# wenet-e2e/wetts

Measured on AMD Instinct MI355X. Metric: audio samples/sec + RTF @22.05 kHz, VITS-Baker, 1/2/4/8 MI355X, higher is better.
Workload: dtype f32

## Files before the change

### wetts_amd/build.py

```python
import hashlib
import os
import subprocess
import sys

HERE = os.path.dirname(os.path.abspath(__file__))
CSRC = os.path.join(HERE, "csrc")
LIBDIR = os.path.join(HERE, "lib")
LIB = os.path.join(LIBDIR, "libwetts_hip.so")
SOURCES = ["conv_mfma.hip", "gemm_pw.hip", "conv_small.hip", "conv_bf16.hip", "resblock16.hip", "resblock2_stage16.hip", "wn16.hip", "qconv_u8.hip", "resblock32.hip", "resblock_chain32.hip", "kernels.hip", "dds_fused.hip", "attention.hip", "mas.hip", "align.hip", "losses.hip", "duration_loss.hip", "stft.hip", "discriminator.hip", "mrd.hip", "model.hip"]
BENCH_SOURCES = ["bench_conv.hip"]
BENCH_LIB = os.path.join(LIBDIR, "libwetts_bench.so")
HEADERS = ["bench_abi.h", "qconv_u8.h", "common.h", "kernels.h", "conv_bf16.h", "conv16_dev.h", "resblock32.h", os.path.join("..", "..", "include", "wetts_hip.h"),
           os.path.join("..", "..", "include", "wetts_vits_model.hpp"),
           os.path.join("..", "..", "tests", "native", "vits_model_main.cpp")]
FLAGS = ["--offload-arch=gfx950", "-O3", "-std=c++17", "-fPIC", "-Wall", "-Wno-unused-function"]


def _hipcc():
    for c in (os.environ.get("HIPCC"), "/opt/rocm/bin/hipcc", "hipcc"):
        if c and (os.path.isabs(c) and os.path.exists(c) or not os.path.isabs(c)):
            return c
    raise RuntimeError("hipcc not found")


def _digest():
    h = hashlib.sha256()
    for f in SOURCES + BENCH_SOURCES + HEADERS:
        with open(os.path.join(CSRC, f), "rb") as fh:
            h.update(fh.read())
    h.update(" ".join(FLAGS).encode())
    return h.hexdigest()


def _obj_digest(src):
    h = hashlib.sha256()
    for f in [src] + [x for x in HEADERS if x.endswith(".h")]:
        with open(os.path.join(CSRC, f), "rb") as fh:
            h.update(fh.read())
    h.update(" ".join(FLAGS).encode())
    return h.hexdigest()


def build(force=False, verbose=True):
    os.makedirs(LIBDIR, exist_ok=True)
    stamp = os.path.join(LIBDIR, "build.sha256")
    dig = _digest()
    if not force and os.path.exists(LIB) and os.path.exists(stamp):
        if open(stamp).read().strip() == dig:
            return LIB
    hipcc = _hipcc()
    objs = []
    procs = []
    for src in SOURCES + BENCH_SOURCES:
        obj = os.path.join(LIBDIR, src.replace(".hip", ".o"))
        objs.append(obj)
        odig = _obj_digest(src)
        ostamp = obj + ".sha256"
        if not force and os.path.exists(obj) and os.path.exists(ostamp) and open(ostamp).read().strip() == odig:
            continue
        if os.path.exists(ostamp):
            os.remove(ostamp)
        cmd = [hipcc] + FLAGS + ["-c", os.path.join(CSRC, src), "-o", obj]
        if verbose:
            print("[wetts_amd.build]", " ".join(cmd), flush=True)
        procs.append((src, ostamp, odig, subprocess.Popen(cmd, stdout=subprocess.PIPE, stderr=subprocess.STDOUT)))
# ... 38 lines not shown
```

### wetts_amd/csrc/common.h

```cpp
#pragma once
#include <hip/hip_runtime.h>
#include <stdint.h>
#include <stdio.h>
#include <string>

#include <string.h>

#include "../../include/wetts_hip.h"

namespace wetts {

void set_error(const char* fmt, ...);

#define WETTS_HIP_CHECK(expr)                                                        \
  do {                                                                               \
    hipError_t _e = (expr);                                                          \
    if (_e != hipSuccess) {                                                          \
      ::wetts::set_error("%s failed: %s (%s:%d)", #expr, hipGetErrorString(_e),      \
                         __FILE__, __LINE__);                                        \
      return WETTS_E_HIP;                                                            \
    }                                                                                \
  } while (0)

static inline bool lds_opt_in(const void* kernel, signed char* state) {
// ... 31 lines not shown
    if (_r != WETTS_OK) return _r; \
  } while (0)

constexpr int kConvCK = 16;

enum InAct { IN_NONE = 0, IN_LRELU = 1 };
enum OutAct { OUT_NONE = 0, OUT_RELU = 1, OUT_GELU = 2, OUT_GATE = 3 };
__device__ __forceinline__ float wn_gate(float ta, float sa) { return tanhf(ta) * (1.f / (1.f + expf(-sa))); }

__device__ __forceinline__ float div_small_const(float v, float d, float c) {
  const float q = v * c;
  const float r = __builtin_fmaf(-d, q, v);
  return __builtin_fmaf(r, c, q);
}

__device__ __forceinline__ bool mrf_div_fast(float d) { return d == 3.f || d == 2.f; }
__device__ __forceinline__ float mrf_div(float v, float d, float dinv, bool fast) {
  return fast ? div_small_const(v, d, dinv) : v / d;
}

struct ConvParams {
  const float* x;
  int64_t x_bs, x_cs;
  int Cin, Tin;
  int vec_in;
  int in_rev_base;
  int in_act;
  float in_slope;
  const float* in_mask;
  int64_t in_mask_stride;
  const float* wpk;
  const float* bias;
  const float* bias_b;
  int64_t bias_b_stride;
  int M, N;
  int ktaps, dil, pad;
  int off_lo, span;
  int nchunks;
  float* out;
  int64_t o_bs, o_cs;
  int Tout;
  int up_shift;
  int up, up_pad;
  int out_act;
  const float* out_mask;
  int64_t out_mask_stride;
  const float* res;
  int64_t r_bs, r_cs;
  int accum;
  float out_div;
  int B;
  int tag;
  int k_rows_padded;
  const int64_t* lens;
  int len_mul;
  float* wn_h;
  float* wn_skip;
  const float* wn_mask;
  int64_t wn_mask_stride;
  int wn_H, wn_last, wn_first;
};

inline ConvParams conv_io(const float* x, int Cin, int T, float* out, int Cout, int B) {
  ConvParams p;
  memset(&p, 0, sizeof(p));
  p.x = x;
  p.x_bs = (int64_t)Cin * T;
  p.x_cs = T;
  p.Tin = T;
  p.in_rev_base = -1;
  p.in_act = IN_NONE;
  p.in_slope = 0.f;
  p.out = out;
  p.o_bs = (int64_t)Cout * T;
  p.o_cs = T;
  p.Tout = T;
  p.out_act = OUT_NONE;
  p.out_div = 1.f;
  p.B = B;
  return p;
}

struct PackedConv {
  float* wpk = nullptr;
  const float* bias = nullptr;
  int M = 0, Cin = 0, ktaps = 0, dil = 1, pad = 0;
  int up = 0, up_pad = 0;
  int Cout = 0;
  int k_orig = 0;
  int off_lo = 0, span = 0, nchunks = 0;
  int gate_H = 0;
};

int32_t pack_conv_weight(const float* w_dev, const float* bias_dev, int Cout, int Cin, int k,
                         int dil, int pad, int transposed, int up, hipStream_t stream,
                         PackedConv* out, int rev_in = 0, int gate_H = 0);
void free_packed(PackedConv* pc);

int32_t launch_conv(const PackedConv& pc, ConvParams p, hipStream_t stream);
bool pw_gemm_eligible(const PackedConv& pc, const ConvParams& p);
int32_t launch_pw_gemm(const PackedConv& pc, const ConvParams& p, hipStream_t stream, int variant);
int32_t launch_conv_group(const PackedConv* const* pcs, const ConvParams* ps, int n, hipStream_t stream,
                          int* launches = nullptr);

int conv_variant();
void set_conv_variant(int v);
int32_t launch_conv_small(const ConvParams& p, hipStream_t stream, bool* taken);
struct SmallConvScope {
  explicit SmallConvScope(int max_tiles);
  ~SmallConvScope();
  int prev;
};

inline int cdiv(int a, int b) { return (a + b - 1) / b; }
inline int64_t align_up(int64_t v, int64_t a) { return (v + a - 1) / a * a; }

inline int device_cus() {
  static int cus = 0;
  if (cus == 0) {
    int dev = 0, n = 0;
    cus = (hipGetDevice(&dev) == hipSuccess &&
           hipDeviceGetAttribute(&n, hipDeviceAttributeMultiprocessorCount, dev) == hipSuccess && n > 0) ? n : 256;
  }
  return cus;
}

}
```

### wetts_amd/csrc/conv_mfma.hip

```cpp
#include <stdlib.h>

#include "common.h"

namespace wetts {

typedef float f32x16 __attribute__((ext_vector_type(16)));
typedef float f32x4v __attribute__((ext_vector_type(4)));
constexpr int kBufRsrcDword3 = 0x00020000;

__device__ __forceinline__ float lrelu2(float x, float slope) {
  const float m = x * slope;
  float r;
  asm("v_max_f32 %0, %1, %2" : "=v"(r) : "v"(x), "v"(m));
  return r;
}

__global__ void pack_conv_weight_kernel(const float* __restrict__ w, float* __restrict__ out,
                                        int M, int Cin, int Cout, int k, int ktaps, int up,
                                        int transposed, int rev_in, int gate_H, int G, int64_t total) {
  int64_t idx = (int64_t)blockIdx.x * blockDim.x + threadIdx.x;
  if (idx >= total) return;
  int s = (int)(idx & 3);
  int lane = (int)((idx >> 2) & 63);
  int64_t rest = idx >> 8;
  int g = (int)(rest % G);
  int mt32 = (int)(rest / G);
  int kstep = g * 4 + s;
  int per_chunk = ktaps * 8;
  int chunk = kstep / per_chunk;
  int within = kstep % per_chunk;
  int tap = within / 8;
  int pair = within % 8;
  int ci = chunk * kConvCK + pair * 2 + (lane >> 5);
  int row = mt32 * 32 + (lane & 31);
  float v = 0.f;
  if (row < M && ci < Cin) {
    if (!transposed) {
      const int src = gate_H > 0 ? (row & 1) * gate_H + (row >> 1) : row;
      v = w[((int64_t)src * Cin + (rev_in ? Cin - 1 - ci : ci)) * k + tap];
    } else {
      int co = row / up, ph = row % up;
      int kk = ph + tap * up;
      if (kk < k) v = w[((int64_t)ci * Cout + co) * k + kk];
    }
  }
  out[idx] = v;
}

int32_t pack_conv_weight(const float* w_dev, const float* bias_dev, int Cout, int Cin, int k,
                         int dil, int pad, int transposed, int up, hipStream_t stream,
                         PackedConv* pc, int rev_in, int gate_H) {
  WETTS_REQUIRE(gate_H == 0 || (!transposed && Cout == 2 * gate_H), "gate packing needs a Conv1d with 2 * gate_H rows");
  pc->gate_H = gate_H;
  pc->Cin = Cin;
  pc->Cout = Cout;
// ... 645 lines not shown
    total += (int64_t)cdiv(gp.p[j].N, NT) * cdiv(gp.p[j].M, MT) * gp.p[j].B;
  }
  gp.first[gp.n] = (int)total;
  WETTS_REQUIRE(total > 0 && total < (1ll << 31), "conv group grid size");
  const size_t lds = (size_t)2 * kConvCK * (conv_has_fixed_stride(NT) ? conv_fixed_stride(NT) : ((NT + max_span + 3 + 3) & ~3)) *
                     sizeof(float);
  hipLaunchKernelGGL((conv_mfma_group_kernel<MB, NB, WM, WN, 1>), dim3((unsigned)total), dim3(256), lds, stream, gp);
  WETTS_LAUNCH_CHECK();
  return WETTS_OK;
}

int32_t launch_conv_group(const PackedConv* const* pcs, const ConvParams* ps, int n, hipStream_t stream,
                          int* launches) {
  if (launches) *launches = n;
  if (n <= 0) return WETTS_OK;
  ConvGroupParams gp;
  memset(&gp, 0, sizeof(gp));
  bool ok = n >= 2 && n <= kConvGroupMax && conv_variant() == 0;
  int order[kConvGroupMax] = {0, 1, 2};
  if (ok) {
    for (int a = 0; a < n; ++a)
      for (int b = a + 1; b < n; ++b)
        if (pcs[order[b]]->ktaps > pcs[order[a]]->ktaps) { int t = order[a]; order[a] = order[b]; order[b] = t; }
  }
  int max_span = 0;
  for (int j = 0; j < n && ok; ++j) {
    gp.p[j] = ps[order[j]];
    WETTS_TRY(prepare_conv(*pcs[order[j]], gp.p[j]));
    const ConvParams& q = gp.p[j];
    ok = q.up == 0 && q.out_act == OUT_NONE && q.out_mask == nullptr && q.out_div == 1.f && q.tag && conv_fast_ok(q) &&
         q.M == gp.p[0].M && q.N == gp.p[0].N && q.B == gp.p[0].B && q.Cin == gp.p[0].Cin && q.lens == gp.p[0].lens;
    if (q.span > max_span) max_span = q.span;
  }
  gp.n = n;
  if (ok) {
    const ConvParams& q = gp.p[0];
    const int64_t cols = (int64_t)q.N * q.B;
    auto nblk = [&](int mt, int nt) { return (int64_t)cdiv(q.M, mt) * cdiv(q.N, nt) * q.B; };
    if (q.M >= 128 && cols >= 4096 && nblk(128, 128) >= 384) {
      if (launches) *launches = 1;
      return launch_group_cfg<1, 4, 4, 1>(gp, max_span, stream);
    }
    if (q.M > 32 && q.M < 128 && cols >= 8192 && nblk(64, 256) >= 384) {
      if (launches) *launches = 1;
      return launch_group_cfg<1, 4, 2, 2>(gp, max_span, stream);
    }
  }
  for (int j = 0; j < n; ++j) WETTS_TRY(launch_conv(*pcs[j], ps[j], stream));
  return WETTS_OK;
}

int32_t launch_conv(const PackedConv& pc, ConvParams p, hipStream_t stream) {
  WETTS_TRY(prepare_conv(pc, p));
  if (conv_variant() == 0 && p.lens == nullptr) {
    bool taken = false;
    WETTS_TRY(launch_conv_small(p, stream, &taken));
    if (taken) return WETTS_OK;
  }
  {
    const int v = conv_variant();
    if ((v == 0 || (v >= 7 && v <= 9)) && pw_gemm_eligible(pc, p)) return launch_pw_gemm(pc, p, stream, v);
  }
  const int64_t cols = (int64_t)p.N * p.B;
  switch (conv_variant()) {
    case 2: return launch_cfg<1, 2, 4, 1>(p, stream);
    case 3: return launch_cfg<1, 4, 2, 2>(p, stream);
    case 4: return launch_cfg<1, 2, 2, 2>(p, stream);
    case 5: return launch_cfg<1, 1, 2, 2>(p, stream);
    case 6: return launch_cfg<1, 4, 4, 1>(p, stream);
    default: break;
  }
  auto nblk = [&](int mt, int nt) { return (int64_t)cdiv(p.M, mt) * cdiv(p.N, nt) * p.B; };
  constexpr int64_t kFill = 384;
  if (p.M >= 128 && cols >= 4096) {
    const int64_t n128 = nblk(128, 128);
    const int kCUs = device_cus();
    if (n128 >= 4 * kCUs) return launch_cfg<1, 4, 4, 1>(p, stream);
    auto cost = [&](int64_t blocks, int area, double eff) {
      return (blocks < kCUs ? 4.0 : 1.0) * (double)((blocks + kCUs - 1) / kCUs) * area / eff;
    };
    const double c128 = cost(n128, 128 * 128, 1.18), c64w = cost(nblk(64, 128), 64 * 128, 1.07),
                 c64 = cost(nblk(64, 64), 64 * 64, 1.0);
    if (c128 <= c64w && c128 <= c64) return launch_cfg<1, 4, 4, 1>(p, stream);
    if (c64w <= c64) return launch_cfg<1, 2, 2, 2>(p, stream);
    return launch_cfg<1, 1, 2, 2>(p, stream);
  }
  if (p.M > 32 && cols >= 8192) {
    if (nblk(64, 256) >= kFill) return launch_cfg<1, 4, 2, 2>(p, stream);
    return launch_cfg<1, 1, 2, 2>(p, stream);
  }
  if (p.M <= 32 && cols >= 8192 && p.ktaps >= 5) return launch_cfg<1, 4, 1, 4>(p, stream);
  if (p.M <= 32 && cols >= 8192) return launch_cfg<1, 2, 1, 4>(p, stream);
  return launch_cfg<1, 1, 2, 2>(p, stream);
}

}
```

### wetts_amd/csrc/gemm_pw.hip

```cpp
#include "common.h"

namespace wetts {

typedef float f32x16 __attribute__((ext_vector_type(16)));
typedef float f32x4v __attribute__((ext_vector_type(4)));
constexpr int kPwRsrcDword3 = 0x00020000;

struct PwParams {
  const float* x;
  int64_t x_bs;
  int x_cs, K, N;
  const float* wpk;
  int64_t wpk_bytes;
  int G;
  const float* bias;
  const float* bias_b;
  int64_t bias_b_stride;
  int M;
  float* out;
  int64_t o_bs;
  int o_cs;
  const float* res;
  int64_t r_bs;
  int r_cs;
// ... 187 lines not shown

template <int CKS, int NBMAX, bool TAG = false>
__global__ __launch_bounds__(256) __attribute__((amdgpu_waves_per_eu(4, 4))) void pw_gemm_kernel(const PwParams p) {
  extern __shared__ __attribute__((aligned(16))) float smem[];
  const int tid = threadIdx.x;
  const int lane = tid & 63;
  const int wave = __builtin_amdgcn_readfirstlane(tid >> 6);
  int bid = blockIdx.x;
  const int total = gridDim.x;
  if ((total & 7) == 0) bid = (bid & 7) * (total >> 3) + (bid >> 3);
  const int part = bid % p.S;
  bid /= p.S;
  const int mtile = bid % p.mtiles;
  const int b = __builtin_amdgcn_readfirstlane(bid / p.mtiles);
  __amdgpu_buffer_rsrc_t rsx = __builtin_amdgcn_make_buffer_rsrc(
      const_cast<float*>(p.x + (int64_t)b * p.x_bs), 0, __builtin_amdgcn_readfirstlane(p.K * p.x_cs * 4), kPwRsrcDword3);
  __amdgpu_buffer_rsrc_t rsw = __builtin_amdgcn_make_buffer_rsrc(const_cast<float*>(p.wpk), 0, (int)p.wpk_bytes,
                                                                 kPwRsrcDword3);
  int u = part * p.upb;
  const int u1 = min(u + p.upb, p.U);
  while (u < u1) {
    const int w = u1 - u;
    if (NBMAX >= 4 && w >= 4) {
      pw_pass<CKS, NBMAX, (NBMAX >= 4 ? 4 : NBMAX)>(p, smem, b, mtile, u * 32, lane, wave, rsx, rsw);
      u += 4;
    } else if (NBMAX >= 2 && w >= 2) {
      pw_pass<CKS, NBMAX, (NBMAX >= 2 ? 2 : NBMAX)>(p, smem, b, mtile, u * 32, lane, wave, rsx, rsw);
      u += 2;
    } else {
      pw_pass<CKS, NBMAX, 1>(p, smem, b, mtile, u * 32, lane, wave, rsx, rsw);
      u += 1;
    }
  }
}

bool pw_gemm_eligible(const PackedConv& pc, const ConvParams& p) {
  if (pc.ktaps != 1 || pc.up != 0 || pc.pad != 0) return false;
  if (p.in_act != IN_NONE || p.in_mask != nullptr || p.in_rev_base >= 0 || p.lens != nullptr) return false;
  if (p.accum || p.out_div != 1.f || p.out_act == OUT_GATE) return false;
  if (p.wn_skip && ((p.wn_H % 32) != 0 || (pc.M % 32) != 0 || p.res || p.out_act != OUT_NONE || p.out_mask ||
                    p.wn_mask_stride < p.Tout))
    return false;
  if (p.res && (p.out_act != OUT_NONE || p.out_mask)) return false;
  if (p.res && (pc.M % 32) != 0) return false;
  if ((int64_t)pc.M * p.o_cs * 4 >= (1ll << 31) || (p.res && (int64_t)pc.M * p.r_cs * 4 >= (1ll << 31))) return false;
  if (((pc.Cin % 16) != 0 && !p.k_rows_padded) || pc.Cin < 32) return false;
  if ((p.x_cs & 3) != 0 || (p.x_bs & 3) != 0 || (reinterpret_cast<uintptr_t>(p.x) & 15) != 0) return false;
  if (p.Tin > p.x_cs || p.x_cs < 4 || p.Tout != p.Tin) return false;
  if ((int64_t)pc.nchunks * 16 * p.x_cs * 4 >= (1ll << 31)) return false;
  if (p.k_rows_padded && p.x_bs < (int64_t)pc.nchunks * 16 * p.x_cs) return false;
  return true;
}

static void pw_schedule(int strips, int U, int K, int slots, int* S_out, int* upb_out) {
  const int cus = device_cus();
  double best = 1e30;
  int bestS = 1;
  for (int S = 1; S <= U; ++S) {
    const int upb = cdiv(U, S);
    if (S > 1 && cdiv(U, S - 1) == upb) continue;
    const int64_t blocks = (int64_t)strips * cdiv(U, upb);
    const int64_t per_cu = cdiv(blocks, cus);
    const int npass = upb / 4 + ((upb % 4) >= 2 ? 1 : 0) + ((upb % 4) & 1);
    double block_cost = (double)upb * K + npass * (0.12 * K + 96.0);
    block_cost += ((upb % 4) >= 2 ? 2.0 * K * 0.08 : 0.0) + ((upb % 4) & 1 ? 1.0 * K * 0.20 : 0.0);
    const int resident = (int)(per_cu < slots ? per_cu : slots);
    const double eff = resident >= 3 ? 1.0 : resident == 2 ? 0.85 : 0.6;
    const double cost = (double)per_cu * block_cost / eff;
    if (cost < best * 0.999) {
      best = cost;
      bestS = cdiv(U, upb);
    }
  }
  *S_out = bestS;
  *upb_out = cdiv(U, bestS);
}

template <int CKS, int NBMAX>
static int32_t launch_pw(const PwParams& p, int64_t blocks, hipStream_t stream, bool tag = false) {
  const size_t lds = PwLds<CKS, NBMAX>::kBytes;
  static signed char opt_in[64] = {};
  if (lds > 64 * 1024 && !lds_opt_in(reinterpret_cast<const void*>(&pw_gemm_kernel<CKS, NBMAX>), opt_in)) {
    set_error("pw_gemm_kernel: the device refused the %zu-byte dynamic LDS opt-in", lds);
    return WETTS_E_HIP;
  }
  if (tag && lds <= 64 * 1024)
    hipLaunchKernelGGL((pw_gemm_kernel<CKS, NBMAX, true>), dim3((unsigned)blocks), dim3(256), lds, stream, p);
  else
    hipLaunchKernelGGL((pw_gemm_kernel<CKS, NBMAX>), dim3((unsigned)blocks), dim3(256), lds, stream, p);
  WETTS_LAUNCH_CHECK();
  return WETTS_OK;
}

int32_t launch_pw_gemm(const PackedConv& pc, const ConvParams& cp, hipStream_t stream, int variant) {
  PwParams p;
  memset(&p, 0, sizeof(p));
  p.x = cp.x;
  p.x_bs = cp.x_bs;
  p.x_cs = (int)cp.x_cs;
  p.K = pc.nchunks * 16;
  p.N = cp.Tout;
  p.wpk = pc.wpk;
  p.G = pc.nchunks * 2;
  p.mtiles = cdiv(pc.M, 128);
  p.wpk_bytes = (int64_t)p.mtiles * 4 * p.G * 1024;
  p.bias = pc.bias;
  p.bias_b = cp.bias_b;
// ... 34 lines not shown
```

### wetts_amd/csrc/model.hip

```cpp
#include <stdarg.h>
#include <stdlib.h>
#include <string.h>

#include <map>
#include <string>
#include <vector>

#include "common.h"
#include "conv_bf16.h"
#include "resblock32.h"
#include "qconv_u8.h"
#include "kernels.h"

namespace wetts {

static thread_local char g_err[512] = "";

void set_error(const char* fmt, ...) {
  va_list ap;
  va_start(ap, fmt);
  vsnprintf(g_err, sizeof(g_err), fmt, ap);
  va_end(ap);
}

struct TensorSpec {
  std::string name;
  int64_t shape[4];
  int64_t offset, numel;
  int dil = 1, pad = 0, transposed = 0, up = 0;
  int bias = -1;
};

struct Layout {
  std::vector<TensorSpec> specs;
  std::map<std::string, int> index;
  int64_t total = 0;
  void add(const std::string& name, int64_t d0, int64_t d1 = 0, int64_t d2 = 0, int64_t d3 = 0) {
    TensorSpec t;
    t.name = name;
    t.shape[0] = d0; t.shape[1] = d1; t.shape[2] = d2; t.shape[3] = d3;
    t.numel = d0 * (d1 ? d1 : 1) * (d2 ? d2 : 1) * (d3 ? d3 : 1);
    t.offset = total;
    total += (t.numel + 63) / 64 * 64;
    index[name] = (int)specs.size();
    specs.push_back(t);
  }
  void add_conv(const std::string& prefix, int Cout, int Cin, int k, int dil = 1, int pad = 0, int transposed = 0,
                int up = 0, bool bias = true) {
    const int w = (int)specs.size();
    add(prefix + ".weight", transposed ? Cin : Cout, transposed ? Cout : Cin, k);
    specs[w].dil = dil; specs[w].pad = pad; specs[w].transposed = transposed; specs[w].up = up;
    if (bias) {
      specs[w].bias = w + 1;
      add(prefix + ".bias", Cout);
    }
  }
  const TensorSpec* find(const std::string& name) const {
    auto it = index.find(name);
    return it == index.end() ? nullptr : &specs[it->second];
  }
};

static const float* tensor(const Layout& L, const float* blob, const std::string& name) {
// ... 306 lines not shown
  PackedConv conv_pre;
  std::vector<PackedConv> ups;
  std::vector<RB> rbs;
  const float* conv_post_w = nullptr;
  const float *dec_cond_w = nullptr, *dec_cond_b = nullptr;
  int hop = 1;
  PackedConv v_in, v_out, v_istft, v_istft_onnx;
  mutable int istft_mode = 0;
  std::vector<ConvNeXt> v_layers;
  const float *v_npre_g = nullptr, *v_npre_b = nullptr, *v_npost_g = nullptr, *v_npost_b = nullptr;
  std::vector<float*> v_owned;
  mutable bool mrf_timing = false;
  mutable std::vector<std::pair<hipEvent_t, hipEvent_t>> mrf_events;
  mutable int64_t mrf_launches = 0;
  mutable int32_t mrf_calls = 0;
  mutable double mrf_bytes = 0;
  mutable int dec_precision = 0;
  mutable int dec_unfused = 0;
  mutable int dec_serial = 0;
  int fuse32_lds = 160 * 1024;
  int fuse32_kmax128 = 11;
  int fuse32_maxc = 32;
  int fuse32_kmax = 99;
  int fuse32_kwide = 3;
  int fuse2_maxc = 128;
  int fuse_min_blocks = 128;
  int small_max_tiles = 256;
  int chain_whole_waste_pct = 15;
  int chain_whole_maxc = 64;
  int chain_pair_maxc = 32;
  int chain_pair_kmax = 3;
  int fuse2_waste_pct = 20;
  mutable int flow_precision = 0;
  mutable std::vector<std::vector<PackedConvB>> b_wn_in, b_wn_rs;
  mutable PackedConvB b_post;
  mutable float* b_post_wpad = nullptr;
  mutable PackedQConv q_pre, q_cond, q_post;
  mutable std::vector<std::vector<PackedQConv>> q_c1, q_c2;
  mutable bool q_packed = false;
  mutable int flow_packed_prec = 0, dec_packed_prec = 0;
  mutable std::vector<PackedConvB> b_ups;
  mutable PackedConvB b_pre;
  mutable std::vector<std::vector<PackedConvB>> b_c1, b_c2;
  mutable int32_t* status_word = nullptr;
  mutable uint64_t rng_seed = 0, rng_offset = 0;
  int mrf_streams = 1;
  int mrf_fork_maxc = 1 << 20;
  int stage2_pct = 30;
  int dds_fused = 1;
  int attn_small_max_t = 128;
  int wn_gate = 1;
  int wn_fuse = 1;
  int small_fork = 1;
  int conv_groups = 1;
  hipStream_t aux_stream[WETTS_MAX_RB_KERNELS] = {};
  hipEvent_t ev_fork = nullptr, ev_chain[WETTS_MAX_RB_KERNELS] = {};
  bool fork_ok = false;

  int spec_channels = 0;
  bool post_loaded = false;
  Layout post_layout;
  float* post_blob = nullptr;
  PackedConv pe_pre, pe_proj;
  std::vector<PackedConv> pe_in, pe_rs, fwd_pre;
  const float *pe_cond_w = nullptr, *pe_cond_b = nullptr;

  bool dur_loaded = false;
  Layout dur_layout;
  float* dur_blob = nullptr;
  ConvFlowW dur_cf1;
  std::vector<ConvFlowW> dur_post_cf;
  const float *dur_post_pre_w = nullptr, *dur_post_pre_b = nullptr;
  PackedConv dur_post_proj;
  DDS dur_post_dds;
  const float *dur_qm = nullptr, *dur_qlogs = nullptr;

  const float* T(const std::string& name) const { return tensor(layout, blob, name); }
};

namespace wetts {

struct Bump {
  char* base;
  int64_t cap, off = 0;
  bool ok = true;
  Bump(void* p, int64_t c) : base((char*)p), cap(c) {}
  template <typename T>
  T* take(int64_t n) {
    int64_t bytes = align_up(n * (int64_t)sizeof(T), 256);
    if (off + bytes > cap) {
      ok = false;
      return nullptr;
    }
    T* r = (T*)(base + off);
    off += bytes;
    return r;
  }
};

struct ConvRef {
  const float *w, *b;
  int Cout, Cin, k, dil, pad, transposed, up;
};

static int32_t find_conv(const Layout& L, const float* blob, const std::string& prefix, ConvRef* r) {
  const std::string wname = prefix + ".weight";
// ... 229 lines not shown
    PackedConv* pc = g.kind == GenConv::PRE  ? &m->conv_pre
                     : g.kind == GenConv::UP ? &m->ups[g.i]
                     : g.kind == GenConv::C1 ? &m->rbs[g.n].c1[g.d]
                     : g.kind == GenConv::C2 ? &m->rbs[g.n].c2[g.d]
                                             : nullptr;
    if (pc) WETTS_TRY(load_conv(m, g.prefix, s, pc));
    if (g.kind == GenConv::UP) m->hop *= g.up;
  }
  m->conv_post_w = m->T("dec.conv_post.weight");
  m->dec_cond_w = m->T("dec.cond.weight");
  m->dec_cond_b = m->T("dec.cond.bias");
  return WETTS_OK;
}

static int64_t A256(int64_t n_floats) { return align_up(n_floats * 4, 256); }

static int64_t ws_encoder(const wetts_config_t* c, int B, int Tx) {
  const int64_t H = c->hidden_channels, F = c->filter_channels, nh = c->n_heads;
  int64_t n = 0;
  n += 5 * A256(B * H * Tx);
  n += A256(B * F * Tx);
  n += A256(B * nh * (int64_t)Tx * Tx + B * H * Tx + B * nh * (2 * c->window_size + 1) * Tx);
  n += A256(B * H * Tx);
  n += A256(B * H);
  return n;
}

static int64_t ws_sdp(const wetts_config_t* c, int B, int Tx) {
  const int64_t H = c->hidden_channels;
  return 5 * A256(B * H * Tx) + A256(B * 32 * Tx) + A256(B * 2 * Tx) + A256(B * H) + 256;
}

static int64_t ws_dp(const wetts_config_t* c, int B, int Tx) {
  const int64_t H = c->hidden_channels, Fd = c->dp_filter_channels;
  return A256(B * H * Tx) + 2 * A256(B * Fd * Tx) + A256(B * H);
}

static int64_t ws_flow(const wetts_config_t* c, int B, int Ty_) {
  const int64_t H = c->hidden_channels, I = c->inter_channels;
  const int64_t Ty = ((int64_t)Ty_ + 3) & ~3ll;
  int64_t n = 3 * A256(B * I * Ty) + A256(B * Ty) + 3 * A256(B * H * Ty) + 2 * A256(B * 2 * H * Ty) +
              A256(B * (I / 2) * Ty) + A256(B * 2 * H * c->flow_wn_layers);
  n += 2 * align_up(B * H * Ty * 2, 256) + 2 * align_up(B * 2 * H * Ty * 2, 256) + A256(B * H * Ty);
  if (c->transformer_flows != 0) {
    const int64_t He = half_enc_flows(c) ? I / 2 : H;
    n += 9 * A256(B * He * Ty) +
         A256(attn_score_elems(half_enc_flows(c) ? -1 : 4, (int)(He / 2), B, 2, Ty) + B * He * Ty +
              (int64_t)B * 2 * 9 * Ty);
  }
  return n;
}

static int64_t dec_max_elems(const wetts_config_t* c, int B, int L) {
  int64_t ch = c->upsample_initial_channel, len = L, mx = (int64_t)B * ch * len;
  for (int i = 0; i < c->n_upsamples; ++i) {
    ch /= 2;
    len *= c->upsample_rates[i];
    int64_t e = (int64_t)B * ch * len;
    if (e > mx) mx = e;
  }
  return mx;
}

static int64_t vocos_fs(int L) { return ((int64_t)L + 1 + 3) & ~3ll; }
static int64_t vocos_rows(const wetts_config_t* c) { return ((int64_t)c->istft_n_fft + 2 + 15) & ~15ll; }

static int64_t ws_vocos(const wetts_config_t* c, int B, int L) {
  const int64_t F = vocos_fs(L), VC = c->vocos_channels, VH = c->vocos_h_channels, NF = c->istft_n_fft;
  return A256(B * c->inter_channels * F) + 3 * A256(B * VC * F) + A256(B * VH * F) +
         A256(B * (NF + 2) * F) + A256(B * vocos_rows(c) * F) + A256(B * NF * F) + A256(B * VC);
}

static int64_t ws_decoder(const wetts_config_t* c, int B, int L) {
  if (c->vocoder_type == 1) return ws_vocos(c, B, L);
  const int64_t f32need = (3 + 3 * (int64_t)c->n_resblock_kernels) * A256(dec_max_elems(c, B, L)) +
                          A256((int64_t)B * c->upsample_initial_channel);
  int64_t lenmax = L;
  for (int i = 0; i < c->n_upsamples; ++i) lenmax *= c->upsample_rates[i];
  const int64_t u8need = 6 * A256(dec_max_elems(c, B, L)) + A256((int64_t)B * c->upsample_initial_channel) +
                         align_up(dec_max_elems(c, B, L) + 32 * (int64_t)B * lenmax, 256) +
                         align_up(4 * (int64_t)B * lenmax, 256) + 2048 + 16384 +
                         align_up((int64_t)B * (lenmax / 128 + 1) * 64, 256);
  return f32need > u8need ? f32need : u8need;
}

static void free_posterior(wetts_model* m) {
  free_packed(&m->pe_pre);
  free_packed(&m->pe_proj);
  for (auto* v : {&m->pe_in, &m->pe_rs, &m->fwd_pre})
    for (PackedConv& pc : *v) free_packed(&pc);
  m->pe_in.clear();
  m->pe_rs.clear();
  m->fwd_pre.clear();
  if (m->post_blob) (void)hipFree(m->post_blob);
  m->post_blob = nullptr;
  m->pe_cond_w = m->pe_cond_b = nullptr;
  m->post_layout = Layout();
  m->post_loaded = false;
}

static void free_dds(DDS* d) {
  for (int i = 0; i < 3; ++i) free_packed(&d->c1x1[i]);
}

static void free_convflow(ConvFlowW* cf) {
  free_dds(&cf->dds);
  free_packed(&cf->proj);
// ... 106 lines not shown
int32_t wetts_duration_blob_tensor_info(const wetts_config_t* cfg, int32_t index, char* name_buf, size_t name_buf_len,
                                        int64_t* offset, int64_t* numel, int64_t shape[4]) {
  WETTS_TRY(validate_config(cfg));
  Layout L;
  build_duration_layout(cfg, L);
  WETTS_REQUIRE(index >= 0 && index < (int32_t)L.specs.size(), "tensor index %d out of range", index);
  const TensorSpec& t = L.specs[index];
  WETTS_REQUIRE(name_buf && name_buf_len > t.name.size(), "name buffer too small");
  strcpy(name_buf, t.name.c_str());
  if (offset) *offset = t.offset;
  if (numel) *numel = t.numel;
  if (shape)
    for (int i = 0; i < 4; ++i) shape[i] = t.shape[i];
  return WETTS_OK;
}

int64_t wetts_duration_blob_numel(const wetts_config_t* cfg) {
  if (validate_config(cfg) != WETTS_OK) return WETTS_E_INVALID;
  Layout L;
  build_duration_layout(cfg, L);
  return L.total;
}

int32_t wetts_create(const wetts_config_t* cfg, const float* blob_dev, int64_t blob_numel,
                     void* stream, wetts_model_t** out) {
  WETTS_TRY(validate_config(cfg));
  WETTS_REQUIRE(out != nullptr && blob_dev != nullptr, "null argument");
  hipStream_t s = (hipStream_t)stream;
  wetts_model* m = new wetts_model();
  m->cfg = *cfg;
  build_layout(cfg, m->layout);
  if (blob_numel != m->layout.total) {
    set_error("blob has %lld floats, layout needs %lld", (long long)blob_numel,
              (long long)m->layout.total);
    delete m;
    return WETTS_E_INVALID;
  }
  hipError_t e = hipMalloc((void**)&m->blob, (size_t)blob_numel * sizeof(float));
  if (e != hipSuccess) {
    set_error("hipMalloc(blob) failed: %s", hipGetErrorString(e));
    delete m;
    return WETTS_E_HIP;
  }
  e = hipMemcpyAsync(m->blob, blob_dev, (size_t)blob_numel * sizeof(float),
                     hipMemcpyDeviceToDevice, s);
  int32_t r = (e == hipSuccess) ? build_model(m, s) : WETTS_E_HIP;
  {
    struct Knob { const char* name; int* field; };
    const Knob knobs[] = {
        {"stage2_pct", &m->stage2_pct}, {"dds_fused", &m->dds_fused}, {"wn_fuse", &m->wn_fuse}, {"wn_gate", &m->wn_gate},
        {"fuse2_waste_pct", &m->fuse2_waste_pct}, {"fuse_min_blocks", &m->fuse_min_blocks},
        {"chain_whole_pct", &m->chain_whole_waste_pct}, {"chain_whole_maxc", &m->chain_whole_maxc},
        {"small_max_tiles", &m->small_max_tiles}, {"attn_small_max_t", &m->attn_small_max_t},
    };
    if (const char* env = getenv("WETTS_TUNE")) {
      std::string all(env);
      size_t pos = 0;
      while (pos < all.size()) {
        size_t end = all.find(',', pos);
        if (end == std::string::npos) end = all.size();
        const std::string item = all.substr(pos, end - pos);
        const size_t eq = item.find('=');
        bool known = false;
        if (eq != std::string::npos)
          for (const Knob& k : knobs)
            if (item.compare(0, eq, k.name) == 0 && strlen(k.name) == eq) {
              *k.field = atoi(item.c_str() + eq + 1);
              known = true;
            }
        if (!known && !item.empty()) {
          set_error("WETTS_TUNE: unknown setting '%s'", item.c_str());
          r = WETTS_E_INVALID;
        }
        pos = end + 1;
      }
    }
    if (r == WETTS_OK && !m->wn_gate) {
      for (int f = 0; f < cfg->flow_n_flows && r == WETTS_OK; ++f)
        for (int i = 0; i < cfg->flow_wn_layers && r == WETTS_OK; ++i) {
          free_packed(&m->flows[f].in_layers[i]);
          r = pack(m->layout, m->blob, S("flow.flows.%d.enc.in_layers.%d", flow_key_stride(cfg) * f, i), s,
                   &m->flows[f].in_layers[i]);
        }
    }
    if (m->mrf_streams < 1) m->mrf_streams = 1;
    if (m->mrf_streams > cfg->n_resblock_kernels) m->mrf_streams = cfg->n_resblock_kernels;
    m->fork_ok = hipEventCreateWithFlags(&m->ev_fork, hipEventDisableTiming) == hipSuccess && m->ev_fork;
    for (int j = 0; j < cfg->n_resblock_kernels; ++j) {
      if (hipEventCreateWithFlags(&m->ev_chain[j], hipEventDisableTiming) != hipSuccess || !m->ev_chain[j]) m->fork_ok = false;
      if (j > 0)
        if (hipStreamCreateWithFlags(&m->aux_stream[j], hipStreamNonBlocking) != hipSuccess || !m->aux_stream[j]) m->fork_ok = false;
    }
    (void)hipGetLastError();
  }
  if (r == WETTS_OK) {
    e = hipStreamSynchronize(s);
    if (e != hipSuccess) {
      set_error("weight packing failed: %s", hipGetErrorString(e));
      r = WETTS_E_HIP;
    }
  }
  if (r != WETTS_OK) {
    wetts_destroy(m);
    return r;
  }
  *out = m;
// ... 1226 lines not shown
        WETTS_TRY(launch_resblock_pair32(rb.c1[d], rb.c2[d], pp, s));
        count(1, 2 + accum);
      } else {
        ConvParams p2 = conv_io(chain_buf[j][2], ch, len, outp[j], ch, B);
        p2.in_act = IN_LRELU;
        p2.in_slope = 0.1f;
        p2.res = rx[j];
        p2.r_bs = (int64_t)ch * len;
        p2.r_cs = len;
        p2.accum = accum;
        p2.out_div = odiv;
        p2.tag = 1;
        p2.lens = lens;
        p2.len_mul = spf;
        if (last_d || m->dec_unfused) {
          WETTS_TRY(launch_conv(rb.c2[d], p2, s));
          count(1, 3 + accum);
        } else {
          g2[n2] = &rb.c2[d];
          p2s[n2++] = p2;
        }
      }
      rx[j] = outp[j];
    }
    if (n2 > 0) {
      int nl = 0;
      WETTS_TRY(launch_conv_group(g2, p2s, n2, s, &nl));
      count(nl, 3.0 * n2);
    }
  }
  return WETTS_OK;
}

static int32_t run_hifigan(const wetts_model* m, const float* z, int64_t z_bs, int64_t z_cs,
                           const float* y_mask, int64_t mask_stride, const float* g, int B, int L,
                           float* audio, void* workspace, int64_t workspace_bytes, hipStream_t s,
                           DecTiming* tm, const int64_t* lens = nullptr) {
  const wetts_config_t* c = &m->cfg;
  const int I = c->inter_channels, C0 = c->upsample_initial_channel;
  const int64_t mx = dec_max_elems(c, B, L);
  Bump ws(workspace, workspace_bytes);
  float* bx = ws.take<float>(mx);
  float* bt = ws.take<float>(mx);
  float* bs = ws.take<float>(mx);
  float* chain_buf[WETTS_MAX_RB_KERNELS][3];
  for (int j = 0; j < c->n_resblock_kernels; ++j)
    for (int q = 0; q < 3; ++q) chain_buf[j][q] = ws.take<float>(mx);
  float* cond = ws.take<float>((int64_t)B * C0);
  if (!ws.ok) {
    set_error("hifigan: workspace too small (need %lld bytes)",
              (long long)ws_decoder(c, B, L));
    return WETTS_E_WORKSPACE;
  }
  {
    ConvParams p = conv_io(z, I, L, bx, C0, B);
    p.x_bs = z_bs;
    p.x_cs = z_cs;
    if (y_mask) {
      p.in_mask = y_mask;
      p.in_mask_stride = mask_stride;
    }
    if (has_g(c) && g) {
      WETTS_TRY(k_cond_linear(g, m->dec_cond_w, m->dec_cond_b, B, C0, c->gin_channels, cond, s));
      p.bias_b = cond;
      p.bias_b_stride = C0;
    }
    p.lens = lens;
    p.len_mul = 1;
    WETTS_TRY(launch_conv(m->conv_pre, p, s));
  }
  int ch = C0, len = L;
  int spf = 1;
  float* x = bx;
  float* xs = bs;
  const int nk = c->n_resblock_kernels, nd = c->n_resblock_dilations;
  for (int i = 0; i < c->n_upsamples; ++i) {
    const int u = c->upsample_rates[i];
    {
      ConvParams p = conv_io(x, ch, len, bt, ch / 2, B);
      p.in_act = IN_LRELU;
      p.in_slope = 0.1f;
      p.Tout = len * u;
      p.o_bs = (int64_t)(ch / 2) * len * u;
      p.o_cs = (int64_t)len * u;
      p.lens = lens;
      p.len_mul = spf;
      WETTS_TRY(launch_conv(m->ups[i], p, s));
    }
    ch /= 2;
    len *= u;
    spf *= u;
    float* xu = bt;
    float* xsum = (x == bx) ? bs : bx;
    (void)xs;
    if (tm && tm->on) WETTS_HIP_CHECK(hipEventRecord(tm->e0, s));
    hipEvent_t lv0 = nullptr, lv1 = nullptr;
    if (m->mrf_timing) {
      WETTS_HIP_CHECK(hipEventCreate(&lv0));
      WETTS_HIP_CHECK(hipEventCreate(&lv1));
      WETTS_HIP_CHECK(hipEventRecord(lv0, s));
    }
    const bool small_stage = !lens && (int64_t)cdiv(ch, 64) * cdiv(len, 64) * B <= m->small_max_tiles;
    const int nstreams = !m->fork_ok ? 1 : (c->resblock == 1 && ((m->small_fork && small_stage) || (ch <= m->mrf_fork_maxc && !m->dec_serial))) ? nk : m->mrf_streams;
    const bool forked = nstreams > 1;
    if (forked) WETTS_HIP_CHECK(hipEventRecord(m->ev_fork, s));
    const bool chain_addr_ok = (int64_t)ch * len * 4 < (int64_t)INT32_MAX;
    const bool grouped = c->resblock == 1 && !forked && m->conv_groups;
    if (grouped) WETTS_TRY(run_stage_rb1_grouped(m, i, xu, xsum, chain_buf, ch, len, spf, B, lens, tm, s));
    for (int j = 0; j < (grouped ? 0 : nk); ++j) {
      const RB& rb = m->rbs[i * nk + j];
      hipStream_t sj = (forked && j > 0 && j < nstreams) ? m->aux_stream[j] : s;
      if (sj != s) WETTS_HIP_CHECK(hipStreamWaitEvent(sj, m->ev_fork, 0));
      float* fa = chain_buf[j][0];
      float* fb = chain_buf[j][1];
      float* ft = chain_buf[j][2];
      const float* rx = xu;
      if (c->resblock == 1 && !m->dec_unfused && nd <= RESCHAIN32_MAX_PAIRS &&
          ch <= m->chain_whole_maxc && m->chain_whole_waste_pct > 0 && len % 4 == 0 && chain_addr_ok &&
          resblock_chain32_supported(rb.c1.data(), rb.c2.data(), nd, m->fuse32_lds / 2,
                                     m->chain_whole_waste_pct)) {
        int dl[RESCHAIN32_MAX_PAIRS];
        for (int d = 0; d < nd; ++d) dl[d] = rb.c1[d].dil;
        if (cdiv(len, resblock_chain32_nto(ch, rb.c1[0].ktaps, dl, nd)) * B >= m->fuse_min_blocks) {
          ResChain32Params cp;
          memset(&cp, 0, sizeof(cp));
          cp.x = rx;
          cp.out = xsum;
          cp.T = len;
          cp.B = B;
          cp.accum = (j > 0) ? 1 : 0;
          cp.out_div = (j == nk - 1) ? (float)nk : 1.f;
          cp.slope = 0.1f;
// ... 922 lines not shown
```

Measured before the change: 52.43 million.

## Add dedicated MFMA transposed-conv upsample kernel with padded pre-conv output

Adds a specialised f32 MFMA kernel for the HiFi-GAN transposed-conv upsample layers (2-tap polyphase, up 2/4/8). It fuses the leaky-ReLU on the input, double-buffers through LDS using buffer-to-LDS loads, and writes the interleaved polyphase output directly. It is used when the generic path would waste tile columns or has unaligned Tin. To allow aligned 16-byte loads, conv_pre output is padded to a multiple of 4 columns and the padding is zeroed by an extra small kernel, which adds one launch and slightly larger workspace.

```diff
diff --git a/wetts_amd/build.py b/wetts_amd/build.py
--- a/wetts_amd/build.py
+++ b/wetts_amd/build.py
@@ -7,10 +7,10 @@
 CSRC = os.path.join(HERE, "csrc")
 LIBDIR = os.path.join(HERE, "lib")
 LIB = os.path.join(LIBDIR, "libwetts_hip.so")
-SOURCES = ["conv_mfma.hip", "gemm_pw.hip", "conv_small.hip", "conv_bf16.hip", "resblock16.hip", "resblock2_stage16.hip", "wn16.hip", "qconv_u8.hip", "resblock32.hip", "resblock_chain32.hip", "kernels.hip", "dds_fused.hip", "attention.hip", "mas.hip", "align.hip", "losses.hip", "duration_loss.hip", "stft.hip", "discriminator.hip", "mrd.hip", "model.hip"]
+SOURCES = ["conv_mfma.hip", "upsample32.hip", "gemm_pw.hip", "conv_small.hip", "conv_bf16.hip", "resblock16.hip", "resblock2_stage16.hip", "wn16.hip", "qconv_u8.hip", "resblock32.hip", "resblock_chain32.hip", "kernels.hip", "dds_fused.hip", "attention.hip", "mas.hip", "align.hip", "losses.hip", "duration_loss.hip", "stft.hip", "discriminator.hip", "mrd.hip", "model.hip"]
 BENCH_SOURCES = ["bench_conv.hip"]
 BENCH_LIB = os.path.join(LIBDIR, "libwetts_bench.so")
-HEADERS = ["bench_abi.h", "qconv_u8.h", "common.h", "kernels.h", "conv_bf16.h", "conv16_dev.h", "resblock32.h", os.path.join("..", "..", "include", "wetts_hip.h"),
+HEADERS = ["bench_abi.h", "qconv_u8.h", "common.h", "kernels.h", "conv_bf16.h", "conv16_dev.h", "resblock32.h", "upsample32.h", os.path.join("..", "..", "include", "wetts_hip.h"),
            os.path.join("..", "..", "include", "wetts_vits_model.hpp"),
            os.path.join("..", "..", "tests", "native", "vits_model_main.cpp")]
 FLAGS = ["--offload-arch=gfx950", "-O3", "-std=c++17", "-fPIC", "-Wall", "-Wno-unused-function"]
diff --git a/wetts_amd/csrc/common.h b/wetts_amd/csrc/common.h
--- a/wetts_amd/csrc/common.h
+++ b/wetts_amd/csrc/common.h
@@ -107,6 +107,8 @@
   int B;
   int tag;
   int k_rows_padded;
+  int in_pad_zeroed;
+  int ups_kernel;
   const int64_t* lens;
   int len_mul;
   float* wn_h;
@@ -155,6 +157,7 @@
 int32_t launch_conv(const PackedConv& pc, ConvParams p, hipStream_t stream);
 bool pw_gemm_eligible(const PackedConv& pc, const ConvParams& p);
 int32_t launch_pw_gemm(const PackedConv& pc, const ConvParams& p, hipStream_t stream, int variant);
+void pw_schedule(int strips, int U, int K, int slots, int* S_out, int* upb_out);
 int32_t launch_conv_group(const PackedConv* const* pcs, const ConvParams* ps, int n, hipStream_t stream,
                           int* launches = nullptr);
 
diff --git a/wetts_amd/csrc/conv_mfma.hip b/wetts_amd/csrc/conv_mfma.hip
--- a/wetts_amd/csrc/conv_mfma.hip
+++ b/wetts_amd/csrc/conv_mfma.hip
@@ -1,6 +1,7 @@
 #include <stdlib.h>
 
 #include "common.h"
+#include "upsample32.h"
 
 namespace wetts {
 
@@ -752,11 +753,16 @@
 
 int32_t launch_conv(const PackedConv& pc, ConvParams p, hipStream_t stream) {
   WETTS_TRY(prepare_conv(pc, p));
+  const bool ups32 = p.ups_kernel > 0 && pc.up > 0 && conv_variant() == 0 && ups32_eligible(pc, p);
+  if (ups32 && p.ups_kernel >= 2) return launch_ups32(pc, p, stream);
   if (conv_variant() == 0 && p.lens == nullptr) {
     bool taken = false;
     WETTS_TRY(launch_conv_small(p, stream, &taken));
     if (taken) return WETTS_OK;
   }
+  if (ups32 && (int64_t)p.N * p.B >= kUps32MinCols &&
+      ((p.Tin & 3) != 0 || (int64_t)cdiv(p.N, 128) * 128 * 100 > (int64_t)p.N * 105 || p.M < 128))
+    return launch_ups32(pc, p, stream);
   {
     const int v = conv_variant();
     if ((v == 0 || (v >= 7 && v <= 9)) && pw_gemm_eligible(pc, p)) return launch_pw_gemm(pc, p, stream, v);
diff --git a/wetts_amd/csrc/gemm_pw.hip b/wetts_amd/csrc/gemm_pw.hip
--- a/wetts_amd/csrc/gemm_pw.hip
+++ b/wetts_amd/csrc/gemm_pw.hip
@@ -263,7 +263,7 @@
   return true;
 }
 
-static void pw_schedule(int strips, int U, int K, int slots, int* S_out, int* upb_out) {
+void pw_schedule(int strips, int U, int K, int slots, int* S_out, int* upb_out) {
   const int cus = device_cus();
   double best = 1e30;
   int bestS = 1;
diff --git a/wetts_amd/csrc/model.hip b/wetts_amd/csrc/model.hip
--- a/wetts_amd/csrc/model.hip
+++ b/wetts_amd/csrc/model.hip
@@ -9,6 +9,7 @@
 #include "common.h"
 #include "conv_bf16.h"
 #include "resblock32.h"
+#include "upsample32.h"
 #include "qconv_u8.h"
 #include "kernels.h"
 
@@ -421,6 +422,7 @@
   int wn_gate = 1;
   int wn_fuse = 1;
   int small_fork = 1;
+  int ups_kernel = 1;
   int conv_groups = 1;
   hipStream_t aux_stream[WETTS_MAX_RB_KERNELS] = {};
   hipEvent_t ev_fork = nullptr, ev_chain[WETTS_MAX_RB_KERNELS] = {};
@@ -756,7 +758,7 @@
 }
 
 static int64_t dec_max_elems(const wetts_config_t* c, int B, int L) {
-  int64_t ch = c->upsample_initial_channel, len = L, mx = (int64_t)B * ch * len;
+  int64_t ch = c->upsample_initial_channel, len = L, mx = (int64_t)B * ch * (((int64_t)L + 3) & ~3ll);
   for (int i = 0; i < c->n_upsamples; ++i) {
     ch /= 2;
     len *= c->upsample_rates[i];
@@ -969,6 +971,7 @@
         {"fuse2_waste_pct", &m->fuse2_waste_pct}, {"fuse_min_blocks", &m->fuse_min_blocks},
         {"chain_whole_pct", &m->chain_whole_waste_pct}, {"chain_whole_maxc", &m->chain_whole_maxc},
         {"small_max_tiles", &m->small_max_tiles}, {"attn_small_max_t", &m->attn_small_max_t},
+        {"ups_kernel", &m->ups_kernel},
     };
     if (const char* env = getenv("WETTS_TUNE")) {
       std::string all(env);
@@ -2301,6 +2304,8 @@
               (long long)ws_decoder(c, B, L));
     return WETTS_E_WORKSPACE;
   }
+  const bool ups32_first = !lens && (m->ups_kernel >= 2 || (m->ups_kernel == 1 && ((int64_t)L + 1) * B >= kUps32MinCols));
+  const int L4 = ups32_first ? (L + 3) & ~3 : L;
   {
     ConvParams p = conv_io(z, I, L, bx, C0, B);
     p.x_bs = z_bs;
@@ -2316,7 +2321,12 @@
     }
     p.lens = lens;
     p.len_mul = 1;
+    if (L4 != L) {
+      p.o_cs = L4;
+      p.o_bs = (int64_t)C0 * L4;
+    }
     WETTS_TRY(launch_conv(m->conv_pre, p, s));
+    if (L4 != L) WETTS_TRY(ups32_zero_pad(bx, (int64_t)B * C0, L, L4, s));
   }
   int ch = C0, len = L;
   int spf = 1;
@@ -2327,6 +2337,12 @@
     const int u = c->upsample_rates[i];
     {
       ConvParams p = conv_io(x, ch, len, bt, ch / 2, B);
+      if (i == 0 && L4 != L) {
+        p.x_cs = L4;
+        p.x_bs = (int64_t)ch * L4;
+        p.in_pad_zeroed = 1;
+      }
+      p.ups_kernel = m->ups_kernel;
       p.in_act = IN_LRELU;
       p.in_slope = 0.1f;
       p.Tout = len * u;
diff --git a/wetts_amd/csrc/upsample32.h b/wetts_amd/csrc/upsample32.h
--- /dev/null
+++ b/wetts_amd/csrc/upsample32.h
@@ -0,0 +1,12 @@
+#pragma once
+#include "common.h"
+
+namespace wetts {
+
+constexpr int64_t kUps32MinCols = 8192;
+
+bool ups32_eligible(const PackedConv& pc, const ConvParams& p);
+int32_t launch_ups32(const PackedConv& pc, const ConvParams& p, hipStream_t stream);
+int32_t ups32_zero_pad(float* x, int64_t rows, int T, int T4, hipStream_t stream);
+
+}
diff --git a/wetts_amd/csrc/upsample32.hip b/wetts_amd/csrc/upsample32.hip
--- /dev/null
+++ b/wetts_amd/csrc/upsample32.hip
@@ -0,0 +1,351 @@
+#include <type_traits>
+
+#include "upsample32.h"
+
+namespace wetts {
+
+typedef float f32x16 __attribute__((ext_vector_type(16)));
+typedef float f32x4v __attribute__((ext_vector_type(4)));
+typedef float f32x4u __attribute__((ext_vector_type(4), aligned(4)));
+typedef float f32x2u __attribute__((ext_vector_type(2), aligned(4)));
+constexpr int kUpsRsrcDword3 = 0x00020000;
+
+struct UpsParams {
+  const float* x;
+  int64_t x_bs;
+  int x_cs, Tin, nch;
+  float slope;
+  const float* wpk;
+  int wpk_bytes;
+  int G;
+  const float* bias;
+  float* out;
+  int64_t o_bs;
+  int o_cs, Tout, N;
+  int up, sh, pad;
+  int S, upb, U, mtiles;
+};
+
+template <int WN>
+struct UpsLds {
+  static constexpr int kW = 128 * WN + 32;
+  static constexpr int kB = kConvCK * kW;
+  static constexpr int kA = (4 / WN) * 4 * 256;
+  static constexpr int kBuf = kB + kA;
+  static constexpr size_t kBytes = (size_t)2 * kBuf * sizeof(float);
+};
+
+__device__ __forceinline__ float ups_lrelu(float x, float slope) {
+  const float m = x * slope;
+  float r;
+  asm("v_max_f32 %0, %1, %2" : "=v"(r) : "v"(x), "v"(m));
+  return r;
+}
+
+template <int WN, int NBP>
+__device__ __forceinline__ void ups_compute(f32x16 (&acc)[NBP], const float* buf, int lane, int wave) {
+  using L = UpsLds<WN>;
+  constexpr int W = L::kW;
+  const int half = lane >> 5, wn = wave % WN;
+  const float* Bb = buf + half * W + wn * (32 * NBP) + (lane & 31) + 4;
+  const float* Ab = buf + L::kB + (wave / WN) * 1024 + lane * 4;
+#pragma unroll
+  for (int g = 0; g < 4; ++g) {
+    const f32x4v a = *reinterpret_cast<const f32x4v*>(Ab + g * 256);
+    const int tap = g >> 1;
+#pragma unroll
+    for (int s = 0; s < 4; ++s) {
+      const int pair = (g & 1) * 4 + s;
+      float bv[NBP];
+#pragma unroll
+      for (int j = 0; j < NBP; ++j) bv[j] = Bb[pair * 2 * W + 32 * j - tap];
+      const float av = s == 0 ? a.x : s == 1 ? a.y : s == 2 ? a.z : a.w;
+#pragma unroll
+      for (int j = 0; j < NBP; ++j) acc[j] = __builtin_amdgcn_mfma_f32_32x32x2f32(av, bv[j], acc[j], 0, 0, 0);
+    }
+  }
+}
+
+template <int NBP>
+__device__ __forceinline__ void ups_store(const UpsParams& p, const f32x16 (&acc)[NBP], char* obase, int rowu, int colw0, int lane) {
+  asm volatile("" : "+s"(rowu));
+  asm volatile("" : "+v"(lane));
+  const int half = lane >> 5, sh = p.sh, um = p.up - 1;
+  float bia[16];
+#pragma unroll
+  for (int r = 0; r < 16; ++r) bia[r] = 0.f;
+  if (p.bias) {
+    const unsigned vb = (unsigned)((4 * half) >> sh) * 4u;
+#pragma unroll
+    for (int r = 0; r < 16; ++r) {
+      const char* sb = reinterpret_cast<const char*>(p.bias + ((rowu >> sh) + (((r & 3) + 8 * (r >> 2)) >> sh)));
+      bia[r] = *reinterpret_cast<const float*>(sb + (size_t)vb);
+    }
+  }
+  const unsigned ocs4 = (unsigned)p.o_cs * 4u;
+  const int col0 = colw0 + (lane & 31);
+  const int tl = (col0 << sh) + ((4 * half) & um) - p.pad;
+  const unsigned voff = (unsigned)((4 * half) >> sh) * ocs4 + (unsigned)(tl * 4 + 32);
+  obase -= 32;
+  const int tlo = (colw0 << sh) - p.pad, thi = ((colw0 + 32 * NBP - 1) << sh) + um - p.pad;
+  if (tlo >= 0 && thi < p.Tout) {
+    if (sh >= 2) {
+#pragma unroll
+      for (int q = 0; q < 4; ++q) {
+        char* rb = obase + (size_t)((unsigned)((rowu + 8 * q) >> sh) * ocs4);
+#pragma unroll
+        for (int j = 0; j < NBP; ++j) {
+          f32x4u v;
+          v.x = acc[j][4 * q] + bia[4 * q];
+          v.y = acc[j][4 * q + 1] + bia[4 * q + 1];
+          v.z = acc[j][4 * q + 2] + bia[4 * q + 2];
+          v.w = acc[j][4 * q + 3] + bia[4 * q + 3];
+          *reinterpret_cast<f32x4u*>(rb + (size_t)(voff + (unsigned)((32 * j) << sh) * 4u)) = v;
+        }
+      }
+    } else {
+#pragma unroll
+      for (int q = 0; q < 4; ++q) {
+#pragma unroll
+        for (int e = 0; e < 2; ++e) {
+          char* rb = obase + (size_t)((unsigned)(((rowu + 8 * q) >> 1) + e) * ocs4);
+#pragma unroll
+          for (int j = 0; j < NBP; ++j) {
+            f32x2u v;
+            v.x = acc[j][4 * q + 2 * e] + bia[4 * q + 2 * e];
+            v.y = acc[j][4 * q + 2 * e + 1] + bia[4 * q + 2 * e + 1];
+            *reinterpret_cast<f32x2u*>(rb + (size_t)(voff + (unsigned)(64 * j) * 4u)) = v;
+          }
+        }
+      }
+    }
+    return;
+  }
+  bool ok[NBP][4];
+#pragma unroll
+  for (int j = 0; j < NBP; ++j)
+#pragma unroll
+    for (int i = 0; i < 4; ++i) {
+      const int t = tl + ((32 * j) << sh) + i;
+      ok[j][i] = t >= 0 && t < p.Tout;
+    }
+  __builtin_amdgcn_sched_barrier(0);
+#pragma unroll
+  for (int q = 0; q < 4; ++q) {
+#pragma unroll
+    for (int e = 0; e < 2; ++e) {
+      char* rb = obase + (size_t)((unsigned)(sh >= 2 ? (rowu + 8 * q) >> sh : ((rowu + 8 * q) >> 1) + e) * ocs4);
+      const int i0 = sh >= 2 ? 2 * e : 0;
+#pragma unroll
+      for (int j = 0; j < NBP; ++j) {
+        const unsigned off = voff + (unsigned)((32 * j) << sh) * 4u + (unsigned)i0 * 4u;
+#pragma unroll
+        for (int i = 0; i < 2; ++i) {
+          const int r = 4 * q + 2 * e + i;
+          const bool k = sh >= 2 ? (e ? ok[j][2 + i] : ok[j][i]) : ok[j][i];
+          if (k) *reinterpret_cast<float*>(rb + (size_t)(off + 4u * i)) = acc[j][r] + bia[r];
+        }
+      }
+    }
+  }
+}
+
+template <int WN>
+__global__ __launch_bounds__(256) __attribute__((amdgpu_waves_per_eu(3))) void ups32_kernel(const UpsParams p) {
+  using L = UpsLds<WN>;
+  constexpr int WM = 4 / WN;
+  constexpr int W = L::kW;
+  constexpr int UC = 32 * WN;
+  constexpr int PPR = 32 * WN;
+  constexpr int RPI = 64 / PPR;
+  constexpr int NI = 4 / RPI;
+  extern __shared__ __attribute__((aligned(16))) float smem[];
+  const int tid = threadIdx.x;
+  const int lane = tid & 63;
+  const int wave = __builtin_amdgcn_readfirstlane(tid >> 6);
+  const int wm = wave / WN, wn = wave % WN;
+  int bid = blockIdx.x;
+  const int total = gridDim.x;
+  if ((total & 7) == 0) bid = (bid & 7) * (total >> 3) + (bid >> 3);
+  const int part = bid % p.S;
+  bid /= p.S;
+  const int mtile = bid % p.mtiles;
+  const int b = __builtin_amdgcn_readfirstlane(bid / p.mtiles);
+  int u = part * p.upb;
+  const int u1 = min(u + p.upb, p.U);
+  if (u >= u1) return;
+
+  __amdgpu_buffer_rsrc_t rsx = __builtin_amdgcn_make_buffer_rsrc(
+      const_cast<float*>(p.x + (int64_t)b * p.x_bs), 0, __builtin_amdgcn_readfirstlane(p.nch * kConvCK * p.x_cs * 4),
+      kUpsRsrcDword3);
+  __amdgpu_buffer_rsrc_t rsw = __builtin_amdgcn_make_buffer_rsrc(const_cast<float*>(p.wpk), 0, p.wpk_bytes, kUpsRsrcDword3);
+
+  const int Tin4 = (p.Tin + 3) & ~3;
+  const int srow = lane / PPR, spiece = lane % PPR;
+  const int vB = (srow * p.x_cs + spiece * 4) * 4;
+  const int vH = lane * p.x_cs * 4;
+  const int sA0 = __builtin_amdgcn_readfirstlane((mtile * WM + wm) * p.G * 1024);
+  f32x4v sreg[NI];
+  float hreg;
+  auto issue = [&](int n0, int c, float* buf) {
+    const bool ok = n0 + spiece * 4 + 4 <= Tin4;
+    const int row0 = c * kConvCK + 4 * wave;
+#pragma unroll
+    for (int i = 0; i < NI; ++i) {
+      const int soff = __builtin_amdgcn_readfirstlane(((row0 + i * RPI) * p.x_cs + n0) * 4);
+      sreg[i] = f32x4v{0.f, 0.f, 0.f, 0.f};
+      if (ok) sreg[i] = __builtin_amdgcn_raw_buffer_load_b128(rsx, vB, soff, 0);
+    }
+    hreg = 0.f;
+    if (lane < 4 && n0 > 0) {
+      const int soff = __builtin_amdgcn_readfirstlane((row0 * p.x_cs + n0 - 1) * 4);
+      hreg = __builtin_bit_cast(float, __builtin_amdgcn_raw_buffer_load_b32(rsx, vH, soff, 0));
+    }
+    float* abuf = buf + L::kB + wm * 1024;
+#pragma unroll
+    for (int g = wn * (4 / WN); g < (wn + 1) * (4 / WN); ++g) {
+      const int soff = __builtin_amdgcn_readfirstlane(sA0 + (c * 4 + g) * 1024);
+      __builtin_amdgcn_raw_ptr_buffer_load_lds(rsw, (__attribute__((address_space(3))) void*)(abuf + g * 256), 16, lane * 16,
+                                               soff, 0, 0);
+    }
+  };
+  auto commit = [&](float* buf) {
+#pragma unroll
+    for (int i = 0; i < NI; ++i) {
+      f32x4v v = sreg[i];
+      v.x = ups_lrelu(v.x, p.slope);
+      v.y = ups_lrelu(v.y, p.slope);
+      v.z = ups_lrelu(v.z, p.slope);
+      v.w = ups_lrelu(v.w, p.slope);
+      *reinterpret_cast<f32x4v*>(buf + (4 * wave + i * RPI + srow) * W + 4 + 4 * spiece) = v;
+    }
+    if (lane < 4) buf[(4 * wave + lane) * W + 3] = ups_lrelu(hreg, p.slope);
+  };
+
+  const int rowu = (mtile * WM + wm) * 32;
+  char* obase = reinterpret_cast<char*>(p.out + (int64_t)b * p.o_bs);
+
+  auto run = [&](auto nbc, int u0, int npass) {
+    constexpr int NBP = decltype(nbc)::value;
+    f32x16 acc[NBP];
+    int pu = u0, c = 0, cur = 0, pend_u = -1;
+    const int uend = u0 + npass * NBP;
+    issue(u0 * UC, 0, smem);
+    commit(smem);
+    bool work = true;
+    for (;;) {
+      float* bufc = smem + cur * L::kBuf;
+      float* bufn = smem + (cur ^ 1) * L::kBuf;
+      __builtin_amdgcn_s_waitcnt(0x0F70);
+      __syncthreads();
+      int un = pu, cn = c + 1;
+      if (cn == p.nch) {
+        cn = 0;
+        un = pu + NBP;
+      }
+      const bool more = work && un < uend;
+      if (more) issue(un * UC, cn, bufn);
+      if (pend_u >= 0) {
+        ups_store<NBP>(p, acc, obase, rowu, pend_u * UC + wn * (32 * NBP), lane);
+        pend_u = -1;
+      }
+      if (!work) break;
+      if (c == 0) {
+#pragma unroll
+        for (int j = 0; j < NBP; ++j)
+#pragma unroll
+          for (int r = 0; r < 16; ++r) acc[j][r] = 0.f;
+      }
+      ups_compute<WN, NBP>(acc, bufc, lane, wave);
+      if (c == p.nch - 1) pend_u = pu;
+      if (more) commit(bufn);
+      work = more;
+      pu = un;
+      c = cn;
+      cur ^= 1;
+    }
+  };
+  const int w = u1 - u;
+  if (w >= 4) run(std::integral_constant<int, 4>(), u, w >> 2);
+  u += w & ~3;
+  if (w & 2) run(std::integral_constant<int, 2>(), u, 1);
+  u += w & 2;
+  if (w & 1) run(std::integral_constant<int, 1>(), u, 1);
+}
+
+__global__ void ups32_zero_pad_kernel(float* x, int64_t rows, int T, int T4) {
+  const int64_t r = (int64_t)blockIdx.x * blockDim.x + threadIdx.x;
+  if (r >= rows) return;
+  for (int t = T; t < T4; ++t) x[r * T4 + t] = 0.f;
+}
+
+int32_t ups32_zero_pad(float* x, int64_t rows, int T, int T4, hipStream_t stream) {
+  if (rows <= 0 || T4 <= T) return WETTS_OK;
+  hipLaunchKernelGGL(ups32_zero_pad_kernel, dim3((unsigned)((rows + 255) / 256)), dim3(256), 0, stream, x, rows, T, T4);
+  WETTS_LAUNCH_CHECK();
+  return WETTS_OK;
+}
+
+bool ups32_eligible(const PackedConv& pc, const ConvParams& p) {
+  if (pc.up != 2 && pc.up != 4 && pc.up != 8) return false;
+  if (pc.ktaps != 2 || pc.up_pad < 0 || pc.up_pad >= pc.up) return false;
+  if (p.in_act != IN_LRELU || p.in_slope < 0.f || p.in_slope > 1.f) return false;
+  if (p.in_mask || p.in_rev_base >= 0 || p.lens || p.bias_b || p.res || p.accum || p.out_mask || p.wn_skip) return false;
+  if (p.out_act != OUT_NONE || p.out_div != 1.f) return false;
+  if ((pc.Cin % kConvCK) != 0 || pc.M < 64 || (pc.M % (pc.M >= 128 ? 128 : 64)) != 0) return false;
+  if (p.Tin <= 0 || p.B <= 0 || p.Tout != p.Tin * pc.up || p.o_cs < p.Tout) return false;
+  const int64_t Tin4 = ((int64_t)p.Tin + 3) & ~3ll;
+  if ((p.x_cs & 3) != 0 || (p.x_bs & 3) != 0 || (reinterpret_cast<uintptr_t>(p.x) & 15) != 0 || p.x_cs < Tin4) return false;
+  if (p.x_bs < (int64_t)pc.Cin * p.x_cs) return false;
+  if ((p.Tin & 3) != 0 && !p.in_pad_zeroed) return false;
+  if ((int64_t)pc.Cin * p.x_cs * 4 >= (1ll << 31) || (int64_t)pc.Cout * p.o_cs * 4 >= (1ll << 31) - 64) return false;
+  if ((int64_t)cdiv(pc.M, 128) * 4 * pc.nchunks * 4 * 1024 >= (1ll << 31)) return false;
+  return true;
+}
+
+template <int WN>
+static int32_t launch_ups(UpsParams& p, int B, int M, hipStream_t stream) {
+  p.mtiles = M / (32 * (4 / WN));
+  p.U = cdiv(p.N, 32 * WN);
+  const int strips = B * p.mtiles;
+  const int slots = (int)(160 * 1024 / UpsLds<WN>::kBytes);
+  pw_schedule(strips, p.U, p.nch * kConvCK * 2, slots, &p.S, &p.upb);
+  if (p.upb > 8) {
+    p.upb = 8;
+    p.S = cdiv(p.U, 8);
+  }
+  const int64_t blocks = (int64_t)strips * p.S;
+  WETTS_REQUIRE(blocks > 0 && blocks < (1ll << 31), "ups32 grid size");
+  const size_t lds = UpsLds<WN>::kBytes;
+  static_assert(UpsLds<WN>::kBytes <= 64 * 1024, "no large-LDS opt-in");
+  hipLaunchKernelGGL((ups32_kernel<WN>), dim3((unsigned)blocks), dim3(256), lds, stream, p);
+  WETTS_LAUNCH_CHECK();
+  return WETTS_OK;
+}
+
+int32_t launch_ups32(const PackedConv& pc, const ConvParams& cp, hipStream_t stream) {
+  UpsParams p;
+  memset(&p, 0, sizeof(p));
+  p.x = cp.x;
+  p.x_bs = cp.x_bs;
+  p.x_cs = (int)cp.x_cs;
+  p.Tin = cp.Tin;
+  p.nch = pc.nchunks;
+  p.slope = cp.in_slope;
+  p.wpk = pc.wpk;
+  p.G = pc.nchunks * 4;
+  p.wpk_bytes = cdiv(pc.M, 128) * 4 * p.G * 1024;
+  p.bias = pc.bias;
+  p.out = cp.out;
+  p.o_bs = cp.o_bs;
+  p.o_cs = (int)cp.o_cs;
+  p.Tout = cp.Tout;
+  p.N = cp.Tin + 1;
+  p.up = pc.up;
+  p.sh = pc.up == 2 ? 1 : pc.up == 4 ? 2 : 3;
+  p.pad = pc.up_pad;
+  if (pc.M >= 128) return launch_ups<1>(p, cp.B, pc.M, stream);
+  return launch_ups<2>(p, cp.B, pc.M, stream);
+}
+
+}
```

Result: no change. 52.49 million (median of 6 runs) (+0.1%).
